# DLR-RM/curvature

Hardware: AMD Instinct MI355X
Metric: KFAC factor-build + invert + sample throughput (higher is better)
Workload: dtype f32

## Files before the change

### curvature_amd/csrc/gemm_nt.h

```cpp
#pragma once
#include "common.h"

namespace curv {

constexpr int GEMM_THREADS = 256;

struct GemmDev {
  const float* A;
  const float* B;
  float* C;
  const float* E;
  const float* F;
  long long a_rs, a_cs;
  long long b_rs, b_cs;
  long long c_rs, c_cs;
  long long e_rs, e_cs;
  long long f_rs, f_cs;
  int M, N, K;
  int epilogue;
  float alpha, beta;
  int tiles_n, tile_base;
  int tm;
  int tri;
  unsigned a_bytes, b_bytes;
// ... 20 lines not shown
typedef __attribute__((address_space(3))) char lds_char_t;

__device__ __forceinline__ void nt_epilogue(const GemmDev& d, int i, int j, float acc) {
  gfl* C = (gfl*)d.C;
  const gfl* E = (const gfl*)d.E;
  const gfl* F = (const gfl*)d.F;
  const int ep = d.epilogue;
  const long long ci = i * d.c_rs + j * d.c_cs;
  float v = d.alpha * acc;
  if (ep == CURV_EPI_SQUARE) v = d.alpha * acc * acc;
  else if (ep == CURV_EPI_MUL_E) v *= E[i * d.e_rs + j * d.e_cs];
  else if (ep == CURV_EPI_ADD_E) v += E[i * d.e_rs + j * d.e_cs];
  else if (ep == CURV_EPI_MUL_E_ADD_F) v = v * E[i * d.e_rs + j * d.e_cs] + F[i * d.f_rs + j * d.f_cs];
  if (d.beta != 0.0f) v += d.beta * C[ci];
  C[ci] = v;
}

__device__ __forceinline__ void gemm_nt_tile(const GemmDev& d, int local, lds_char_t* lds, float* __restrict__ slabs) {
  using namespace nt;
  const int tid = threadIdx.x, lane = tid & 63;
  const int wave = __builtin_amdgcn_readfirstlane(tid >> 6);
  const int r32 = lane & 31, h = lane >> 5;
  const int wm = wave >> 1, wn = wave & 1;
  const bool split = d.n_slices > 1;
  const int item = local;
  int slice = 0;
  if (split) { slice = local % d.n_slices; local /= d.n_slices; }
  int tm = local / d.tiles_n, tn = local - tm * d.tiles_n;
  if (d.tri == CURV_TRI_A_LOWER) tm = (d.M + TM - 1) / TM - 1 - tm;
  else if (d.tri == CURV_TRI_B_UPPER) tn = d.tiles_n - 1 - tn;
  const int i0 = tm * TM, j0 = tn * TM, M = d.M, N = d.N;
  int K = d.K;
  const bool cut = (d.tri == CURV_TRI_A_LOWER && i0 + TM < K) || (d.tri == CURV_TRI_B_UPPER && j0 + TM < K);
  if (d.tri == CURV_TRI_A_LOWER) K = min(K, i0 + TM);
  else if (d.tri == CURV_TRI_B_UPPER) K = min(K, j0 + TM);
  int kb = 0;
  bool inner = false;
  if (split) {
    kb = slice * d.kslice;
    if (kb >= K) return;
    inner = kb + d.kslice < K;
    K = min(K, kb + d.kslice);
  }
  (void)cut; (void)inner;
  const int n_stages = (K - kb + KC - 1) / KC;

  const int rsub = RPP * wave + (lane >> LANES_PER_ROW_SHIFT);
  const int g_lane = (lane & (SLOTS - 1)) ^ ((rsub >> KEY_SHIFT) & (SLOTS - 1));
  int voff_a[PIECES], voff_b[PIECES];
#pragma unroll
  for (int p = 0; p < PIECES; ++p) {
    const int ra = min(i0 + 4 * RPP * p + rsub, M - 1), rb = min(j0 + 4 * RPP * p + rsub, N - 1);
    voff_a[p] = (int)(((long long)ra * d.a_rs + 4 * g_lane) * 4);
    voff_b[p] = (int)(((long long)rb * d.b_cs + 4 * g_lane) * 4);
  }
  const __amdgpu_buffer_rsrc_t rsa = __builtin_amdgcn_make_buffer_rsrc((void*)d.A, 0, d.a_bytes, 0x00020000);
  const __amdgpu_buffer_rsrc_t rsb = __builtin_amdgcn_make_buffer_rsrc((void*)d.B, 0, d.b_bytes, 0x00020000);

  unsigned addr[4][STEPS];
#pragma unroll
  for (int o = 0; o < 4; ++o) {
    const int R = ((o < 2) ? 64 * wm : 64 * wn) + (o & 1) * 32 + r32;
    const unsigned pbase = (o < 2) ? 0u : 2u * PANEL_B;
    const int rkey = (R >> KEY_SHIFT) & (SLOTS - 1);
#pragma unroll
    for (int j = 0; j < STEPS; ++j) addr[o][j] = pbase + R * ROW_B + (((2 * j + h) ^ rkey) << 4);
  }
  f32x16 c00 = {0}, c01 = {0}, c10 = {0}, c11 = {0};

  constexpr int OOB = (int)0x80000000;
  auto issue = [&](int i, bool live, int k0n, unsigned nbuf) {
    const int p = i / PIECES, slot = i % PIECES;
    const unsigned lbase = (p ? 2u * PANEL_B : 0u) + nbuf + (unsigned)(RPP * wave + 4 * RPP * slot) * ROW_B;
    if (p == 0) __builtin_amdgcn_raw_ptr_buffer_load_lds(rsa, (lds_void_t*)(lds + lbase), 16, live ? voff_a[slot] : OOB, k0n * 4, 0, 0);
    else __builtin_amdgcn_raw_ptr_buffer_load_lds(rsb, (lds_void_t*)(lds + lbase), 16, live ? voff_b[slot] : OOB, k0n * 4, 0, 0);
  };
  if (n_stages > 0) {
    const bool live = kb + 4 * g_lane < K;
#pragma unroll
    for (int i = 0; i < NP; ++i) issue(i, live, kb, 0u);
  }
  for (int t = 0; t < n_stages; ++t) {
    __builtin_amdgcn_s_waitcnt(0x0f70);
    __syncthreads();
    const bool more = t + 1 < n_stages;
    const int k0n = kb + (t + 1) * KC;
    const bool live_n = more && k0n + 4 * g_lane < K;
    const unsigned buf = (unsigned)(t & 1) * PANEL_B, nbuf = PANEL_B - buf;
    const int kbase = kb + t * KC;
    const bool tail_stage = kbase + KC > K;
    auto rd = [&](int o, int j) { return *reinterpret_cast<const __attribute__((address_space(3))) f32x4*>(lds + addr[o][j] + buf); };
    auto mask_step = [&](int j, f32x4& xa0, f32x4& xa1, f32x4& xb0, f32x4& xb1) {
      if (tail_stage) {
        asm volatile("; k tail" ::: "memory");
#pragma unroll
        for (int e = 0; e < 4; ++e) {
          const bool gone = kbase + 4 * (2 * j + h) + e >= K;
          xa0[e] = gone ? 0.0f : xa0[e]; xa1[e] = gone ? 0.0f : xa1[e];
          xb0[e] = gone ? 0.0f : xb0[e]; xb1[e] = gone ? 0.0f : xb1[e];
        }
      }
    };
    f32x4 a0 = rd(0, 0), a1 = rd(1, 0), b0 = rd(2, 0), b1 = rd(3, 0);
#pragma unroll
    for (int j = 0; j < STEPS; ++j) {
      mask_step(j, a0, a1, b0, b1);
      f32x4 na0, na1, nb0, nb1;
      if (j + 1 < STEPS) { na0 = rd(0, j + 1); na1 = rd(1, j + 1); nb0 = rd(2, j + 1); nb1 = rd(3, j + 1); }
#pragma unroll
      for (int e = 0; e < 4; ++e) {
        c00 = __builtin_amdgcn_mfma_f32_32x32x2f32(a0[e], b0[e], c00, 0, 0, 0);
        c01 = __builtin_amdgcn_mfma_f32_32x32x2f32(a0[e], b1[e], c01, 0, 0, 0);
        c10 = __builtin_amdgcn_mfma_f32_32x32x2f32(a1[e], b0[e], c10, 0, 0, 0);
        c11 = __builtin_amdgcn_mfma_f32_32x32x2f32(a1[e], b1[e], c11, 0, 0, 0);
        if (e < PPS && PPS * j + e < NP) issue(PPS * j + e, live_n, k0n, nbuf);
      }
      if (j + 1 < STEPS) { a0 = na0; a1 = na1; b0 = nb0; b1 = nb1; }
    }
  }

  if (split) {
    gfl* slab = (gfl*)slabs + d.slab_base + (long long)item * (TM * TM);
    auto store_raw = [&](const f32x16& acc, int m, int n) {
      const int c = 64 * wn + 32 * n + r32;
#pragma unroll
      for (int reg = 0; reg < 16; ++reg) {
        const int r = 64 * wm + 32 * m + (reg & 3) + 8 * (reg >> 2) + 4 * h;
        slab[r * TM + c] = acc[reg];
      }
    };
    store_raw(c00, 0, 0);
    store_raw(c01, 0, 1);
    store_raw(c10, 1, 0);
    store_raw(c11, 1, 1);
// ... 18 lines not shown
```

### curvature_amd/csrc/invert.hip

```cpp
#include <type_traits>
#include "kernarg.h"
#include "mma64.h"
#include <hip/hip_ext.h>

#include <algorithm>
#include <chrono>
#include <cstdlib>
#include <mutex>
#include <vector>

namespace curv {

constexpr int INV_THREADS = MMA_THREADS;
constexpr int SQ_FLAGS = 32;
constexpr int SQ_FD = 0, SQ_FLC = 4, SQ_FLROW = 8, SQ_FT = 12;
constexpr int SQ_SPIN_LIMIT = 1 << 21;
#ifdef CURV_SQ_TRACE
__device__ long long g_sq_trace[256];
#define KT_BEGIN(slot) { if (threadIdx.x == 0 && k0 == 4 * (CURV_SQ_TRACE - 1)) atomicMax((unsigned long long*)&g_sq_trace[slot], (1ull << 62) - (unsigned long long)wall_clock64()); }
#define KT_END(slot) { if (threadIdx.x == 0 && k0 == 4 * (CURV_SQ_TRACE - 1)) atomicMax((unsigned long long*)&g_sq_trace[slot], (unsigned long long)wall_clock64()); }
#define SQT(slot) { if (threadIdx.x == 0 && f == 0 && stamp == CURV_SQ_TRACE) g_sq_trace[slot] = wall_clock64(); }
#define FIT(k) { if (threadIdx.x == 0 && trace_base >= 0) g_sq_trace[trace_base + (k)] = wall_clock64(); }
#else
#define SQT(slot)
// ... 5 lines not shown
#define PQT(slot) { if (threadIdx.x == 0 && blockIdx.x == 0 && k0 == 4 * (CURV_SQ_TRACE - 1)) g_sq_trace[slot] = wall_clock64(); }
#else
#define PQT(slot)
#endif

struct InvDev {
  const float* F;
  float* L;
  double* W;
  double* X;
  int* info;
  int n, np, P;
  float sqrt_s, sqrt_n;
  int reverse;
  int f64_in;
  double* Xout;
  const double* R;
  double* Zm;
  int r_minus, pad_;
  float* C32;
  float* X32;
  float* S32;
  double pivot_min;
};
typedef __attribute__((address_space(1))) float gfloat;
__device__ __host__ __forceinline__ bool s_in_sweep(const InvDev& d) { return d.X32 == nullptr; }
__device__ __host__ __forceinline__ int s_kind(const InvDev& d) { return d.X32 != nullptr ? 0 : (d.Zm != nullptr ? 2 : 1); }

template <typename CountFn>
__device__ __forceinline__ bool locate(const InvDev* __restrict__ t, int nf, int bid, CountFn cnt, int& f,
                                       int& local) {
  const int lane = threadIdx.x & 63;
  int base = 0;
  for (int f0 = 0; f0 < nf; f0 += 64) {
    const int ff = f0 + lane;
    const int c = (ff < nf) ? cnt(t[ff]) : 0;
    int incl = c;
#pragma unroll
    for (int o = 1; o < 64; o <<= 1) {
      const int v = __shfl_up(incl, o, 64);
      if (lane >= o) incl += v;
    }
// ... 1038 lines not shown
  if (local < n_below) panel_quarter_body<true>(d, k0, nb, kend + local, 0, q, Own, Ts);
  else panel_quarter_body<false>(d, k0, nb, 0, local - n_below, q, Own, Ts);
  KT_END(237)
}
__global__ void __launch_bounds__(INV_THREADS, 3)
panel_product_kernel(const InvDev* __restrict__ t, int nf, int k0, int kend) {
  __shared__ double As[NB * OPA], Bs[NB * OPA > OKS * LDA ? NB * OPA : OKS * LDA];
  panel_product_body<2>(t, nf, k0, kend, As, Bs);
}
__global__ void __launch_bounds__(1024)
panel_product_wide_kernel(const InvDev* __restrict__ t, int nf, int k0, int kend) {
  __shared__ double As[NB * OPA], Bs[NB * OPA > OKS * LDA ? NB * OPA : OKS * LDA];
  panel_product_body<4>(t, nf, k0, kend, As, Bs);
}

constexpr int SKS = 32;
constexpr int SPA = SKS + 1;
constexpr int SPB = NB + 32;
struct Tile32 {
  const gbyte* a;
  const gbyte* b;
  gfloat* out;
  int np, ke0, ke1;
  bool a64, b64, accumulate, negate;
};
__device__ __forceinline__ void tile32(const Tile32& o, float* __restrict__ As, float* __restrict__ Bs) {
  const int np = o.np;
  const int tid = threadIdx.x, lane = tid & 63, wave = tid >> 6, wm = wave >> 1, wn = wave & 1;
  const int l32 = lane & 31, h = lane >> 5;
  const long long a_off = (long long)(tid >> 3) * np + 4 * (tid & 7), a_step = 32ll * np;
  const long long b_off = (long long)(tid >> 4) * np + 4 * (tid & 15), b_step = 16ll * np;
  typedef const __attribute__((address_space(1))) f32x4 gf4;
  typedef const __attribute__((address_space(1))) f64x4 gd4;
  f32x4 ra[2], rb[2];
  auto fetch = [&](int ke) __attribute__((always_inline)) {
    if (o.a64) {
#pragma unroll
      for (int u = 0; u < 2; ++u) {
        const f64x4 v = *(gd4*)(o.a + (a_off + u * a_step + ke) * 8);
        ra[u] = f32x4{(float)v[0], (float)v[1], (float)v[2], (float)v[3]};
      }
    } else {
#pragma unroll
      for (int u = 0; u < 2; ++u) ra[u] = *(gf4*)(o.a + (a_off + u * a_step + ke) * 4);
    }
    if (o.b64) {
#pragma unroll
      for (int u = 0; u < 2; ++u) {
        const f64x4 v = *(gd4*)(o.b + (b_off + u * b_step + (long long)ke * np) * 8);
        rb[u] = f32x4{(float)v[0], (float)v[1], (float)v[2], (float)v[3]};
      }
    } else {
#pragma unroll
      for (int u = 0; u < 2; ++u) rb[u] = *(gf4*)(o.b + (b_off + u * b_step + (long long)ke * np) * 4);
    }
  };
  f32x16 acc = {0};
  fetch(o.ke0);
  for (int ke = o.ke0; ke < o.ke1; ke += SKS) {
#pragma unroll
    for (int u = 0; u < 2; ++u)
#pragma unroll
      for (int e = 0; e < 4; ++e) {
        As[((tid >> 3) + 32 * u) * SPA + 4 * (tid & 7) + e] = ra[u][e];
        Bs[((tid >> 4) + 16 * u) * SPB + 4 * (tid & 15) + e] = rb[u][e];
      }
    __syncthreads();
    if (ke + SKS < o.ke1) fetch(ke + SKS);
#pragma unroll
    for (int kk = 0; kk < SKS; kk += 2) {
      const float av = As[(32 * wm + l32) * SPA + kk + h];
      const float bv = Bs[(kk + h) * SPB + 32 * wn + l32];
      acc = __builtin_amdgcn_mfma_f32_32x32x2f32(av, bv, acc, 0, 0, 0);
    }
    __syncthreads();
  }
  gbyte* base = (gbyte*)(o.out + (long long)(32 * wm + 4 * h) * np + 32 * wn + l32);
  if (!o.accumulate) {
#pragma unroll
    for (int reg = 0; reg < 16; ++reg)
      *(gfloat*)(base + (long long)((reg & 3) + 8 * (reg >> 2)) * np * 4) = o.negate ? -acc[reg] : acc[reg];
  } else {
    float old[16];
#pragma unroll
    for (int reg = 0; reg < 16; ++reg) old[reg] = *(const gfloat*)(base + (long long)((reg & 3) + 8 * (reg >> 2)) * np * 4);
#pragma unroll
    for (int reg = 0; reg < 16; ++reg) *(gfloat*)(base + (long long)((reg & 3) + 8 * (reg >> 2)) * np * 4) = old[reg] + acc[reg];
  }
}
__device__ __host__ __forceinline__ long long supd_tiles(int P, int kind, int kend) {
  if (kind != 0 || P <= kend) return 0;
  const long long nsb = (P - kend + SB - 1) / SB, ncb = (kend + SB - 1) / SB;
  return nsb * ncb * (SB * SB);
}
__global__ void __launch_bounds__(INV_THREADS, 3)
supd32_kernel(const InvDev* __restrict__ t, int nf, int k0, int kend, int n_items) {
  __shared__ float As[NB * SPA], Bs[SKS * SPB];
  int item;
  {
    const int bid = blockIdx.x, xcd = bid & 7, jj = bid >> 3;
    item = ((jj / (SB * SB)) * 8 + xcd) * (SB * SB) + (jj % (SB * SB));
  }
  if (item >= n_items) return;
  int f, local;
  if (!locate(t, nf, item, [kend](const InvDev& d) { return (int)supd_tiles(d.P, s_kind(d), kend); }, f, local)) return;
  const InvDev& d = t[f];
  const int np = d.np, r = d.P - kend;
  const int ncb = (kend + SB - 1) / SB;
  const int sb = local / (SB * SB), in = local - sb * (SB * SB);
  const int a = sb / ncb, cb = sb - a * ncb;
  const int ri = a * SB + in / SB, j = cb * SB + in % SB;
  if (ri >= r || j >= kend) return;
  const int i = kend + ri;
  const bool own = j >= k0;
  Tile32 o;
  o.np = np;
  o.a = (const gbyte*)((const gfloat*)d.C32 + (long long)i * NB * np);
  o.a64 = false;
  o.b = own ? (const gbyte*)((const gdouble*)d.X + j * NB) : (const gbyte*)((const gfloat*)d.X32 + j * NB);
  o.b64 = own;
  o.ke0 = (own ? j : k0) * NB;
  o.ke1 = kend * NB;
  o.out = (gfloat*)d.S32 + (long long)i * NB * np + j * NB;
  o.accumulate = !own;
  o.negate = false;
  tile32(o, As, Bs);
}
__device__ __host__ __forceinline__ long long xrow_tiles(int P, int kind, int k0, int kend) {
  if (kind != 0 || P <= k0) return 0;
  return (long long)((kend < P ? kend : P) - k0) * k0;
}
__global__ void __launch_bounds__(INV_THREADS, 3)
xrows32_kernel(const InvDev* __restrict__ t, int nf, int k0, int kend) {
  __shared__ float As[NB * SPA], Bs[SKS * SPB];
  int f, local;
  if (!locate(t, nf, blockIdx.x, [k0, kend](const InvDev& d) { return (int)xrow_tiles(d.P, s_kind(d), k0, kend); }, f, local)) return;
  const InvDev& d = t[f];
  const int np = d.np, nb = (kend < d.P ? kend : d.P) - k0;
  const int j = local / nb, c = nb - 1 - (local - j * nb);
  Tile32 o;
  o.np = np;
  o.a = (const gbyte*)((const gdouble*)d.X + (long long)(k0 + c) * NB * np);
  o.a64 = true;
  o.b = (const gbyte*)((const gfloat*)d.S32 + j * NB);
  o.b64 = false;
  o.ke0 = k0 * NB;
  o.ke1 = (k0 + c + 1) * NB;
  o.out = (gfloat*)d.X32 + (long long)(k0 + c) * NB * np + j * NB;
  o.accumulate = false;
  o.negate = true;
  tile32(o, As, Bs);
}

__global__ void __launch_bounds__(INV_THREADS)
inv_finalize_kernel(const InvDev* __restrict__ t, int nf, int sq) {
  __shared__ float tile[NB][NB + 1];
  int f, local;
  if (!locate(t, nf, blockIdx.x, [](const InvDev& d) { return d.P * d.P; }, f, local)) return;
  const InvDev& d = t[f];
  const int n = d.n, np = d.np, q = d.P;
  const int ti = local / q, tj = local - ti * q;
  const gdouble* X = (const gdouble*)d.X;
  const gfloat* X32 = (const gfloat*)d.X32;
  gfloat* L = (gfloat*)d.L;
  const int w = __builtin_amdgcn_readfirstlane(threadIdx.x >> 6), c = threadIdx.x & 63;
  if (!d.reverse) {
    gdouble* Xo = (gdouble*)d.Xout;
    const gdouble* S = d.Zm != nullptr ? (const gdouble*)d.Zm : X;
#pragma unroll 4
    for (int u = 0; u < 16; ++u) {
      const int i = ti * NB + w + 4 * u, j = tj * NB + c;
      if (i < n && j < n) {
        double v = (j <= i) ? S[(long long)i * np + j] : 0.0;
        if (d.r_minus && j <= i) v = ((const gdouble*)d.R)[(long long)i * n + j] - v;
        Xo[(long long)i * n + j] = v;
      }
    }
    return;
  }
  if (tj > ti) {
#pragma unroll 4
    for (int u = 0; u < 16; ++u) {
      const int i = ti * NB + w + 4 * u, j = tj * NB + c;
      if (i < n && j < n) L[(long long)i * n + j] = 0.0f;
    }
    return;
  }
  double xv[16];
  const int i_l = ti * NB + c;
#pragma unroll
  for (int u = 0; u < 16; ++u) {
    const int j = tj * NB + w + 4 * u;
    const int rs = n - 1 - j, cs = n - 1 - i_l;
    const bool live = i_l < n && j < n && j <= i_l;
    if (X32 == nullptr || rs / sq == cs / sq) xv[u] = live ? X[(long long)rs * np + cs] : 0.0;
    else xv[u] = live ? (double)X32[(long long)rs * np + cs] : 0.0;
  }
#pragma unroll
  for (int u = 0; u < 16; ++u) tile[w + 4 * u][c] = (float)xv[u];
  __syncthreads();
#pragma unroll
  for (int u = 0; u < 16; ++u) {
    const int i = ti * NB + w + 4 * u, j = tj * NB + c;
    if (i < n && j < n) L[(long long)i * n + j] = tile[c][w + 4 * u];
  }
}

constexpr int INV_UPLOAD_CHUNK = 28;

static size_t inv_table_bytes(int n) { return align_up((size_t)std::max(n, 1) * sizeof(InvDev), 256); }
static size_t inv_flags_bytes(int n) { return align_up((size_t)std::max(n, 1) * SQ_FLAGS * sizeof(int), 256); }

struct SideStream {
  hipStream_t stream = nullptr;
  hipEvent_t ev_main[2] = {nullptr, nullptr};
  hipEvent_t ev_side[2] = {nullptr, nullptr};
  hipEvent_t ev_tail = nullptr;
};
struct StreamSet {
  SideStream side[2];
  hipStream_t aux = nullptr;
  hipStream_t masked = nullptr;
  hipEvent_t ev_fork = nullptr, ev_join = nullptr, ev_join2 = nullptr;
  hipEvent_t ev_chain[2] = {nullptr, nullptr};
};
// ... 78 lines not shown
extern "C" int curv_debug_sq_trace(long long* out) {
  return hipMemcpyFromSymbol(out, HIP_SYMBOL(curv::g_sq_trace), 256 * sizeof(long long)) == hipSuccess ? 0 : 1;
}
#endif

extern "C" int curv_init_streams(void) {
  StreamSet* ss = nullptr;
  return stream_set(&ss);
}

extern "C" size_t curv_chol_inv_workspace_bytes(const curv_inv_desc* descs, int n_factors) {
  size_t total = 2 * inv_table_bytes(n_factors) + 2 * inv_flags_bytes(n_factors);
  for (int i = 0; i < n_factors; ++i) {
    if (descs[i].n <= 0) return 0;
    const size_t np = (size_t)cdiv(descs[i].n, NB) * NB;
    total += 2 * np * np * sizeof(double) + 3 * np * np * sizeof(float);
  }
  return total;
}

static int sweep_nbo(bool latency_bound) { return latency_bound ? 4 : 6; }
struct GroupSweep {
  hipStream_t stream;
  SideStream* side;
  const std::vector<InvDev>* tabp;
  InvDev* table;
  int* flags;
  bool latency_bound;
  int n_factors = 0, Pmax = 0, NBO = 4, k0 = 0, panel = 0;
  long long fin_tiles = 0, quarter_prod = 0;
  bool use_square = false, far_pending = false, inv_pending = false, capturing = false;
// ... 60 lines not shown
    }
    auto launch_product = [&](hipStream_t st, long long jobs, hipEvent_t done) -> int {
      const InvDev* tb = table;
      if (jobs <= quarter_prod)
        hipExtLaunchKernelGGL(panel_product_quarter_kernel, dim3((unsigned)(cdivll(jobs, 8) * 32)), dim3(INV_THREADS), 0, st,
                              nullptr, done, 0, tb, n_factors, k0, kend);
      else if (jobs <= WIDE_PROD)
        hipExtLaunchKernelGGL(panel_product_wide_kernel, dim3((unsigned)jobs), dim3(1024), 0, st, nullptr, done, 0, tb, n_factors,
                              k0, kend);
      else
        hipExtLaunchKernelGGL(panel_product_kernel, dim3((unsigned)jobs), dim3(INV_THREADS), 0, st, nullptr, done, 0, tb,
                              n_factors, k0, kend);
      CURV_LAUNCH_CHECK();
      return CURV_OK;
    };
    long long inv_jobs = 0, inv_tiles = 0;
    for (const InvDev& d : tab) {
      prod_tiles += panel_jobs(d.P, s_kind(d), k0, kend);
      inv_jobs += xrow_tiles(d.P, s_kind(d), k0, kend);
      inv_tiles += supd_tiles(d.P, s_kind(d), kend);
    }
    bool fork_recorded = false;
    if (prod_tiles > 0) {
      fork_recorded = !capturing;
      const int rc = launch_product(stream, prod_tiles, fork_recorded ? side->ev_main[panel & 1] : nullptr);
      if (rc != CURV_OK) return rc;
    }
    long long near_tiles = 0, far_tiles = 0;
    for (const InvDev& d : tab) {
      near_tiles += strip_tiles(d.P, kend, kend, row0, s_in_sweep(d));
      far_tiles += outer_tiles(d.P, kend, row0, s_in_sweep(d));
    }
    hipStream_t inv_st = side->stream;
    const bool inv_work = inv_jobs > 0 || inv_tiles > 0;
    const bool side_work = far_tiles > 0 || inv_work;
    if (side_work) {
      if (!fork_recorded) CURV_HIP_CHECK(hipEventRecord(side->ev_main[panel & 1], stream));
      CURV_HIP_CHECK(hipStreamWaitEvent(side->stream, side->ev_main[panel & 1], 0));
    }
    if (near_tiles > 0) {
      if (far_pending) {
        CURV_HIP_CHECK(hipStreamWaitEvent(stream, side->ev_side[(panel + 1) & 1], 0));
      }
      far_pending = false;
      if (near_tiles <= WIDE_NEAR)
        hipLaunchKernelGGL(outer_update_wide_kernel, dim3((unsigned)near_tiles), dim3(1024), 0, stream, table, n_factors,
                           k0, kend, kend, row0, 1, (int)near_tiles);
      else
        hipLaunchKernelGGL(outer_update_kernel, dim3((unsigned)near_tiles), dim3(INV_THREADS), 0, stream, table, n_factors, k0,
// ... 9 lines not shown
      if (trail > 0) {
        const long long g1 = cdivll(trail, 8 * SB * SB) * 8 * SB * SB;
        hipExtLaunchKernelGGL(outer_update_dma_kernel, dim3((unsigned)g1), dim3(INV_THREADS), 0, side->stream, nullptr,
                              (ride && s_tiles == 0) ? side->ev_side[panel & 1] : nullptr, 0, tb, n_factors, k0, kend, row0, (int)trail);
        CURV_LAUNCH_CHECK();
      }
      if (s_tiles > 0) {
        const long long g2 = cdivll(s_tiles, 8 * SB * SB) * 8 * SB * SB;
        hipExtLaunchKernelGGL(outer_update_kernel, dim3((unsigned)g2), dim3(INV_THREADS), 0, side->stream, nullptr,
                              ride ? side->ev_side[panel & 1] : nullptr, 0, tb, n_factors, k0, kend, row0, 0, 2, (int)s_tiles);
        CURV_LAUNCH_CHECK();
      }
      if (!ride) CURV_HIP_CHECK(hipEventRecord(side->ev_side[panel & 1], side->stream));
      far_pending = true;
    }
    if (inv_jobs > 0) {
      hipLaunchKernelGGL(xrows32_kernel, dim3((unsigned)inv_jobs), dim3(INV_THREADS), 0, inv_st, table, n_factors, k0, kend);
      CURV_LAUNCH_CHECK();
      inv_pending = true;
    }
    if (inv_tiles > 0) {
      const long long grid = cdivll(inv_tiles, 8 * SB * SB) * 8 * SB * SB;
      hipLaunchKernelGGL(supd32_kernel, dim3((unsigned)grid), dim3(INV_THREADS), 0, inv_st, table, n_factors, k0, kend,
                         (int)inv_tiles);
      CURV_LAUNCH_CHECK();
      inv_pending = true;
    }
    k0 += NBO;
    ++panel;
    return CURV_OK;
  }

  int end(hipEvent_t chain_done = nullptr) {
    if (chain_done != nullptr) CURV_HIP_CHECK(hipEventRecord(chain_done, stream));
    if (far_pending) CURV_HIP_CHECK(hipStreamWaitEvent(stream, side->ev_side[(panel + 1) & 1], 0));
    if (inv_pending) {
      CURV_HIP_CHECK(hipEventRecord(side->ev_tail, side->stream));
      CURV_HIP_CHECK(hipStreamWaitEvent(stream, side->ev_tail, 0));
    }
    hipLaunchKernelGGL(inv_finalize_kernel, dim3((unsigned)fin_tiles), dim3(INV_THREADS), 0, stream, table, n_factors, NBO * NB);
    CURV_LAUNCH_CHECK();
    return CURV_OK;
  }
};

static int chol_sweep_group(hipStream_t stream, SideStream* side, const std::vector<InvDev>& tab, InvDev* table, int* flags,
                            bool latency_bound, hipEvent_t chain_done = nullptr) {
  GroupSweep g(stream, side, tab, table, flags, latency_bound);
  int rc = g.begin();
  while (rc == CURV_OK && !g.done()) rc = g.panel_step();
  return rc == CURV_OK ? g.end(chain_done) : rc;
}

constexpr int SPLIT_P = 16;

// ... 1 lines not shown

static int await_verdict(const EarlyStatus* early) {
  if (early != nullptr) CURV_HIP_CHECK(hipEventSynchronize(early->ev));
  return CURV_OK;
}

static int chol_sweep(hipStream_t stream, std::vector<InvDev>& tab, void* workspace, size_t workspace_bytes,
                      const char* who, const EarlyStatus* early = nullptr) {
  const int n_factors = (int)tab.size();
  static const int latency_max = getenv("CURV_LATENCY_MAX") ? atoi(getenv("CURV_LATENCY_MAX")) : 64;
  bool any_rhs = false;
  for (const InvDev& d : tab) any_rhs = any_rhs || d.R != nullptr;
  const bool latency_bound = n_factors <= latency_max && !any_rhs;
  size_t need = 2 * inv_table_bytes(n_factors) + 2 * inv_flags_bytes(n_factors);
  for (const InvDev& d : tab)
    need += (d.R != nullptr ? 3 : 2) * (size_t)d.np * d.np * sizeof(double) + (d.reverse ? 3 * (size_t)d.np * d.np * sizeof(float) : 0);
  if (workspace == nullptr || workspace_bytes < need) {
    set_error("%s: workspace too small (%zu < %zu bytes)", who, workspace_bytes, need);
    return CURV_ERR_WORKSPACE;
  }
  char* p = reinterpret_cast<char*>(workspace) + 2 * inv_table_bytes(n_factors);
  int* flags0 = reinterpret_cast<int*>(p);
  int* flags1 = reinterpret_cast<int*>(p + inv_flags_bytes(n_factors));
  p += 2 * inv_flags_bytes(n_factors);
  std::vector<InvDev> big, small;
  int Pmax = 0;
  for (const InvDev& d : tab) Pmax = std::max(Pmax, d.P);
  const int split = std::max(SPLIT_P, Pmax / 2);
  for (InvDev& d : tab) {
    d.W = reinterpret_cast<double*>(p); p += (size_t)d.np * d.np * sizeof(double);
    d.X = reinterpret_cast<double*>(p); p += (size_t)d.np * d.np * sizeof(double);
    if (d.R != nullptr) { d.Zm = reinterpret_cast<double*>(p); p += (size_t)d.np * d.np * sizeof(double); }
    if (d.reverse) {
      d.C32 = reinterpret_cast<float*>(p); p += (size_t)d.np * d.np * sizeof(float);
      d.X32 = reinterpret_cast<float*>(p); p += (size_t)d.np * d.np * sizeof(float);
      d.S32 = reinterpret_cast<float*>(p); p += (size_t)d.np * d.np * sizeof(float);
    }
    (d.P > split || latency_bound ? big : small).push_back(d);
  }
  StreamSet* ss = nullptr;
  { const int rc = stream_set(&ss); if (rc != CURV_OK) return rc; }
  InvDev* table0 = reinterpret_cast<InvDev*>(workspace);
  InvDev* table1 = reinterpret_cast<InvDev*>(reinterpret_cast<char*>(workspace) + inv_table_bytes(n_factors));
  hipStreamCaptureStatus capture = hipStreamCaptureStatusNone;
  CURV_HIP_CHECK(hipStreamIsCapturing(stream, &capture));
  if (capture != hipStreamCaptureStatusNone) {
    if (early != nullptr) {
      set_error("%s: the early status read-back is a host copy and cannot be captured", who);
      return CURV_ERR_INVALID;
    }
    if (!big.empty()) {
// ... 144 lines not shown
```

Before: 4204.

## Reuse NT MFMA GEMM stage loop for f32 inverse panel updates

Pulls the double-buffered DMA-to-LDS MFMA stage loop out of the NT GEMM into a shared helper. The inverse's row and Schur-update kernels (tile32-based xrows32/supd32) are replaced with 128x128 NT tiles that work on transposed f32 copies (XT32, ST32), with XCD-aware block ordering. A new xsq32 kernel converts and transposes each diagonal block square into an extra f32 buffer. The finalize kernel now reads the transposed f32 inverse directly, dropping its LDS transpose. The aim is to replace the small 64x64 tiles that use scalar LDS staging with the faster GEMM engine, at the cost of an extra kernel launch and more workspace.

New measurement: 4166. About the same (-0.9%).

```diff
diff --git a/curvature_amd/csrc/gemm_nt.h b/curvature_amd/csrc/gemm_nt.h
--- a/curvature_amd/csrc/gemm_nt.h
+++ b/curvature_amd/csrc/gemm_nt.h
@@ -58,6 +58,85 @@
   else if (ep == CURV_EPI_MUL_E_ADD_F) v = v * E[i * d.e_rs + j * d.e_cs] + F[i * d.f_rs + j * d.f_cs];
   if (d.beta != 0.0f) v += d.beta * C[ci];
   C[ci] = v;
+}
+
+__device__ __forceinline__ void nt_dma_lane(int wave, int lane, int& rsub, int& g_lane) {
+  using namespace nt;
+  rsub = RPP * wave + (lane >> LANES_PER_ROW_SHIFT);
+  g_lane = (lane & (SLOTS - 1)) ^ ((rsub >> KEY_SHIFT) & (SLOTS - 1));
+}
+
+__device__ __forceinline__ void nt_stage_loop(const __amdgpu_buffer_rsrc_t rsa, const __amdgpu_buffer_rsrc_t rsb,
+                                              const int (&voff_a)[nt::PIECES], const int (&voff_b)[nt::PIECES], int g_lane,
+                                              int kb, int K, lds_char_t* lds, f32x16& c00, f32x16& c01, f32x16& c10,
+                                              f32x16& c11) {
+  using namespace nt;
+  const int tid = threadIdx.x, lane = tid & 63;
+  const int wave = __builtin_amdgcn_readfirstlane(tid >> 6);
+  const int r32 = lane & 31, h = lane >> 5;
+  const int wm = wave >> 1, wn = wave & 1;
+  const int n_stages = (K - kb + KC - 1) / KC;
+  unsigned addr[4][STEPS];
+#pragma unroll
+  for (int o = 0; o < 4; ++o) {
+    const int R = ((o < 2) ? 64 * wm : 64 * wn) + (o & 1) * 32 + r32;
+    const unsigned pbase = (o < 2) ? 0u : 2u * PANEL_B;
+    const int rkey = (R >> KEY_SHIFT) & (SLOTS - 1);
+#pragma unroll
+    for (int j = 0; j < STEPS; ++j) addr[o][j] = pbase + R * ROW_B + (((2 * j + h) ^ rkey) << 4);
+  }
+  c00 = f32x16{0}; c01 = f32x16{0}; c10 = f32x16{0}; c11 = f32x16{0};
+
+  constexpr int OOB = (int)0x80000000;
+  auto issue = [&](int i, bool live, int k0n, unsigned nbuf) {
+    const int p = i / PIECES, slot = i % PIECES;
+    const unsigned lbase = (p ? 2u * PANEL_B : 0u) + nbuf + (unsigned)(RPP * wave + 4 * RPP * slot) * ROW_B;
+    if (p == 0) __builtin_amdgcn_raw_ptr_buffer_load_lds(rsa, (lds_void_t*)(lds + lbase), 16, live ? voff_a[slot] : OOB, k0n * 4, 0, 0);
+    else __builtin_amdgcn_raw_ptr_buffer_load_lds(rsb, (lds_void_t*)(lds + lbase), 16, live ? voff_b[slot] : OOB, k0n * 4, 0, 0);
+  };
+  if (n_stages > 0) {
+    const bool live = kb + 4 * g_lane < K;
+#pragma unroll
+    for (int i = 0; i < NP; ++i) issue(i, live, kb, 0u);
+  }
+  for (int t = 0; t < n_stages; ++t) {
+    __builtin_amdgcn_s_waitcnt(0x0f70);
+    __syncthreads();
+    const bool more = t + 1 < n_stages;
+    const int k0n = kb + (t + 1) * KC;
+    const bool live_n = more && k0n + 4 * g_lane < K;
+    const unsigned buf = (unsigned)(t & 1) * PANEL_B, nbuf = PANEL_B - buf;
+    const int kbase = kb + t * KC;
+    const bool tail_stage = kbase + KC > K;
+    auto rd = [&](int o, int j) { return *reinterpret_cast<const __attribute__((address_space(3))) f32x4*>(lds + addr[o][j] + buf); };
+    auto mask_step = [&](int j, f32x4& xa0, f32x4& xa1, f32x4& xb0, f32x4& xb1) {
+      if (tail_stage) {
+        asm volatile("; k tail" ::: "memory");
+#pragma unroll
+        for (int e = 0; e < 4; ++e) {
+          const bool gone = kbase + 4 * (2 * j + h) + e >= K;
+          xa0[e] = gone ? 0.0f : xa0[e]; xa1[e] = gone ? 0.0f : xa1[e];
+          xb0[e] = gone ? 0.0f : xb0[e]; xb1[e] = gone ? 0.0f : xb1[e];
+        }
+      }
+    };
+    f32x4 a0 = rd(0, 0), a1 = rd(1, 0), b0 = rd(2, 0), b1 = rd(3, 0);
+#pragma unroll
+    for (int j = 0; j < STEPS; ++j) {
+      mask_step(j, a0, a1, b0, b1);
+      f32x4 na0, na1, nb0, nb1;
+      if (j + 1 < STEPS) { na0 = rd(0, j + 1); na1 = rd(1, j + 1); nb0 = rd(2, j + 1); nb1 = rd(3, j + 1); }
+#pragma unroll
+      for (int e = 0; e < 4; ++e) {
+        c00 = __builtin_amdgcn_mfma_f32_32x32x2f32(a0[e], b0[e], c00, 0, 0, 0);
+        c01 = __builtin_amdgcn_mfma_f32_32x32x2f32(a0[e], b1[e], c01, 0, 0, 0);
+        c10 = __builtin_amdgcn_mfma_f32_32x32x2f32(a1[e], b0[e], c10, 0, 0, 0);
+        c11 = __builtin_amdgcn_mfma_f32_32x32x2f32(a1[e], b1[e], c11, 0, 0, 0);
+        if (e < PPS && PPS * j + e < NP) issue(PPS * j + e, live_n, k0n, nbuf);
+      }
+      if (j + 1 < STEPS) { a0 = na0; a1 = na1; b0 = nb0; b1 = nb1; }
+    }
+  }
 }
 
 __device__ __forceinline__ void gemm_nt_tile(const GemmDev& d, int local, lds_char_t* lds, float* __restrict__ slabs) {
@@ -87,10 +166,8 @@
     K = min(K, kb + d.kslice);
   }
   (void)cut; (void)inner;
-  const int n_stages = (K - kb + KC - 1) / KC;
-
-  const int rsub = RPP * wave + (lane >> LANES_PER_ROW_SHIFT);
-  const int g_lane = (lane & (SLOTS - 1)) ^ ((rsub >> KEY_SHIFT) & (SLOTS - 1));
+  int rsub, g_lane;
+  nt_dma_lane(wave, lane, rsub, g_lane);
   int voff_a[PIECES], voff_b[PIECES];
 #pragma unroll
   for (int p = 0; p < PIECES; ++p) {
@@ -101,67 +178,8 @@
   const __amdgpu_buffer_rsrc_t rsa = __builtin_amdgcn_make_buffer_rsrc((void*)d.A, 0, d.a_bytes, 0x00020000);
   const __amdgpu_buffer_rsrc_t rsb = __builtin_amdgcn_make_buffer_rsrc((void*)d.B, 0, d.b_bytes, 0x00020000);
 
-  unsigned addr[4][STEPS];
-#pragma unroll
-  for (int o = 0; o < 4; ++o) {
-    const int R = ((o < 2) ? 64 * wm : 64 * wn) + (o & 1) * 32 + r32;
-    const unsigned pbase = (o < 2) ? 0u : 2u * PANEL_B;
-    const int rkey = (R >> KEY_SHIFT) & (SLOTS - 1);
-#pragma unroll
-    for (int j = 0; j < STEPS; ++j) addr[o][j] = pbase + R * ROW_B + (((2 * j + h) ^ rkey) << 4);
-  }
-  f32x16 c00 = {0}, c01 = {0}, c10 = {0}, c11 = {0};
-
-  constexpr int OOB = (int)0x80000000;
-  auto issue = [&](int i, bool live, int k0n, unsigned nbuf) {
-    const int p = i / PIECES, slot = i % PIECES;
-    const unsigned lbase = (p ? 2u * PANEL_B : 0u) + nbuf + (unsigned)(RPP * wave + 4 * RPP * slot) * ROW_B;
-    if (p == 0) __builtin_amdgcn_raw_ptr_buffer_load_lds(rsa, (lds_void_t*)(lds + lbase), 16, live ? voff_a[slot] : OOB, k0n * 4, 0, 0);
-    else __builtin_amdgcn_raw_ptr_buffer_load_lds(rsb, (lds_void_t*)(lds + lbase), 16, live ? voff_b[slot] : OOB, k0n * 4, 0, 0);
-  };
-  if (n_stages > 0) {
-    const bool live = kb + 4 * g_lane < K;
-#pragma unroll
-    for (int i = 0; i < NP; ++i) issue(i, live, kb, 0u);
-  }
-  for (int t = 0; t < n_stages; ++t) {
-    __builtin_amdgcn_s_waitcnt(0x0f70);
-    __syncthreads();
-    const bool more = t + 1 < n_stages;
-    const int k0n = kb + (t + 1) * KC;
-    const bool live_n = more && k0n + 4 * g_lane < K;
-    const unsigned buf = (unsigned)(t & 1) * PANEL_B, nbuf = PANEL_B - buf;
-    const int kbase = kb + t * KC;
-    const bool tail_stage = kbase + KC > K;
-    auto rd = [&](int o, int j) { return *reinterpret_cast<const __attribute__((address_space(3))) f32x4*>(lds + addr[o][j] + buf); };
-    auto mask_step = [&](int j, f32x4& xa0, f32x4& xa1, f32x4& xb0, f32x4& xb1) {
-      if (tail_stage) {
-        asm volatile("; k tail" ::: "memory");
-#pragma unroll
-        for (int e = 0; e < 4; ++e) {
-          const bool gone = kbase + 4 * (2 * j + h) + e >= K;
-          xa0[e] = gone ? 0.0f : xa0[e]; xa1[e] = gone ? 0.0f : xa1[e];
-          xb0[e] = gone ? 0.0f : xb0[e]; xb1[e] = gone ? 0.0f : xb1[e];
-        }
-      }
-    };
-    f32x4 a0 = rd(0, 0), a1 = rd(1, 0), b0 = rd(2, 0), b1 = rd(3, 0);
-#pragma unroll
-    for (int j = 0; j < STEPS; ++j) {
-      mask_step(j, a0, a1, b0, b1);
-      f32x4 na0, na1, nb0, nb1;
-      if (j + 1 < STEPS) { na0 = rd(0, j + 1); na1 = rd(1, j + 1); nb0 = rd(2, j + 1); nb1 = rd(3, j + 1); }
-#pragma unroll
-      for (int e = 0; e < 4; ++e) {
-        c00 = __builtin_amdgcn_mfma_f32_32x32x2f32(a0[e], b0[e], c00, 0, 0, 0);
-        c01 = __builtin_amdgcn_mfma_f32_32x32x2f32(a0[e], b1[e], c01, 0, 0, 0);
-        c10 = __builtin_amdgcn_mfma_f32_32x32x2f32(a1[e], b0[e], c10, 0, 0, 0);
-        c11 = __builtin_amdgcn_mfma_f32_32x32x2f32(a1[e], b1[e], c11, 0, 0, 0);
-        if (e < PPS && PPS * j + e < NP) issue(PPS * j + e, live_n, k0n, nbuf);
-      }
-      if (j + 1 < STEPS) { a0 = na0; a1 = na1; b0 = nb0; b1 = nb1; }
-    }
-  }
+  f32x16 c00, c01, c10, c11;
+  nt_stage_loop(rsa, rsb, voff_a, voff_b, g_lane, kb, K, lds, c00, c01, c10, c11);
 
   if (split) {
     gfl* slab = (gfl*)slabs + d.slab_base + (long long)item * (TM * TM);
diff --git a/curvature_amd/csrc/invert.hip b/curvature_amd/csrc/invert.hip
--- a/curvature_amd/csrc/invert.hip
+++ b/curvature_amd/csrc/invert.hip
@@ -1,4 +1,5 @@
 #include <type_traits>
+#include "gemm_nt.h"
 #include "kernarg.h"
 #include "mma64.h"
 #include <hip/hip_ext.h>
@@ -43,18 +44,21 @@
   float sqrt_s, sqrt_n;
   int reverse;
   int f64_in;
-  double* Xout;
+  union {
+    double* Xout;
+    float* Xsq32;
+  };
   const double* R;
   double* Zm;
   int r_minus, pad_;
   float* C32;
-  float* X32;
-  float* S32;
+  float* XT32;
+  float* ST32;
   double pivot_min;
 };
 typedef __attribute__((address_space(1))) float gfloat;
-__device__ __host__ __forceinline__ bool s_in_sweep(const InvDev& d) { return d.X32 == nullptr; }
-__device__ __host__ __forceinline__ int s_kind(const InvDev& d) { return d.X32 != nullptr ? 0 : (d.Zm != nullptr ? 2 : 1); }
+__device__ __host__ __forceinline__ bool s_in_sweep(const InvDev& d) { return d.XT32 == nullptr; }
+__device__ __host__ __forceinline__ int s_kind(const InvDev& d) { return d.XT32 != nullptr ? 0 : (d.Zm != nullptr ? 2 : 1); }
 
 template <typename CountFn>
 __device__ __forceinline__ bool locate(const InvDev* __restrict__ t, int nf, int bid, CountFn cnt, int& f,
@@ -1123,154 +1127,160 @@
   panel_product_body<4>(t, nf, k0, kend, As, Bs);
 }
 
-constexpr int SKS = 32;
-constexpr int SPA = SKS + 1;
-constexpr int SPB = NB + 32;
-struct Tile32 {
-  const gbyte* a;
-  const gbyte* b;
-  gfloat* out;
-  int np, ke0, ke1;
-  bool a64, b64, accumulate, negate;
+namespace inv32 {
+constexpr int TB = nt::TM / NB;
+constexpr int XCH = 8;
+enum { STORE = 0, STORE_NEG = 1, ADD = 2 };
+struct Panel {
+  const float* base;
+  int pitch;
+  int rows;
+  int row_floats;
 };
-__device__ __forceinline__ void tile32(const Tile32& o, float* __restrict__ As, float* __restrict__ Bs) {
-  const int np = o.np;
-  const int tid = threadIdx.x, lane = tid & 63, wave = tid >> 6, wm = wave >> 1, wn = wave & 1;
-  const int l32 = lane & 31, h = lane >> 5;
-  const long long a_off = (long long)(tid >> 3) * np + 4 * (tid & 7), a_step = 32ll * np;
-  const long long b_off = (long long)(tid >> 4) * np + 4 * (tid & 15), b_step = 16ll * np;
-  typedef const __attribute__((address_space(1))) f32x4 gf4;
-  typedef const __attribute__((address_space(1))) f64x4 gd4;
-  f32x4 ra[2], rb[2];
-  auto fetch = [&](int ke) __attribute__((always_inline)) {
-    if (o.a64) {
-#pragma unroll
-      for (int u = 0; u < 2; ++u) {
-        const f64x4 v = *(gd4*)(o.a + (a_off + u * a_step + ke) * 8);
-        ra[u] = f32x4{(float)v[0], (float)v[1], (float)v[2], (float)v[3]};
-      }
-    } else {
-#pragma unroll
-      for (int u = 0; u < 2; ++u) ra[u] = *(gf4*)(o.a + (a_off + u * a_step + ke) * 4);
-    }
-    if (o.b64) {
-#pragma unroll
-      for (int u = 0; u < 2; ++u) {
-        const f64x4 v = *(gd4*)(o.b + (b_off + u * b_step + (long long)ke * np) * 8);
-        rb[u] = f32x4{(float)v[0], (float)v[1], (float)v[2], (float)v[3]};
-      }
-    } else {
-#pragma unroll
-      for (int u = 0; u < 2; ++u) rb[u] = *(gf4*)(o.b + (b_off + u * b_step + (long long)ke * np) * 4);
-    }
+}
+__device__ __forceinline__ int inv32_item() {
+  const int bid = blockIdx.x, xcd = bid & 7, jj = bid >> 3;
+  return ((jj / inv32::XCH) * 8 + xcd) * inv32::XCH + jj % inv32::XCH;
+}
+static long long inv32_grid(long long items) { return cdivll(items, 8 * inv32::XCH) * 8 * inv32::XCH; }
+__device__ __forceinline__ void inv32_tile(const inv32::Panel& rows, const inv32::Panel& cols, int kb, int K,
+                                           gfloat* __restrict__ out, int out_pitch, int mode, lds_char_t* lds) {
+  using namespace nt;
+  const int tid = threadIdx.x, lane = tid & 63;
+  const int wave = __builtin_amdgcn_readfirstlane(tid >> 6);
+  const int r32 = lane & 31, h = lane >> 5, wm = wave >> 1, wn = wave & 1;
+  int rsub, g_lane;
+  nt_dma_lane(wave, lane, rsub, g_lane);
+  int voff_a[PIECES], voff_b[PIECES];
+#pragma unroll
+  for (int p = 0; p < PIECES; ++p) {
+    const int ra = min(4 * RPP * p + rsub, cols.rows - 1), rb = min(4 * RPP * p + rsub, rows.rows - 1);
+    voff_a[p] = (ra * cols.pitch + 4 * g_lane) * 4;
+    voff_b[p] = (rb * rows.pitch + 4 * g_lane) * 4;
+  }
+  const unsigned a_bytes = (unsigned)(((long long)(cols.rows - 1) * cols.pitch + cols.row_floats) * 4);
+  const unsigned b_bytes = (unsigned)(((long long)(rows.rows - 1) * rows.pitch + rows.row_floats) * 4);
+  const __amdgpu_buffer_rsrc_t rsa = __builtin_amdgcn_make_buffer_rsrc((void*)cols.base, 0, a_bytes, 0x00020000);
+  const __amdgpu_buffer_rsrc_t rsb = __builtin_amdgcn_make_buffer_rsrc((void*)rows.base, 0, b_bytes, 0x00020000);
+  f32x16 c00, c01, c10, c11;
+  nt_stage_loop(rsa, rsb, voff_a, voff_b, g_lane, kb, K, lds, c00, c01, c10, c11);
+  typedef __attribute__((address_space(1))) f32x4 gf4;
+  auto put = [&](const f32x16& acc, int m, int n) {
+    const int c = 64 * wm + 32 * m + 4 * h;
+    if (64 * wm + 32 * m >= cols.rows) return;
+    gfloat* p = out + (long long)(64 * wn + 32 * n + r32) * out_pitch + c;
+    f32x4 v[4];
+#pragma unroll
+    for (int g = 0; g < 4; ++g) v[g] = f32x4{acc[4 * g], acc[4 * g + 1], acc[4 * g + 2], acc[4 * g + 3]};
+    if (mode == inv32::ADD) {
+      f32x4 old[4];
+#pragma unroll
+      for (int g = 0; g < 4; ++g) old[g] = *(const gf4*)(p + 8 * g);
+#pragma unroll
+      for (int g = 0; g < 4; ++g) v[g] = old[g] + v[g];
+    } else if (mode == inv32::STORE_NEG) {
+#pragma unroll
+      for (int g = 0; g < 4; ++g) v[g] = -v[g];
+    }
+#pragma unroll
+    for (int g = 0; g < 4; ++g) *(gf4*)(p + 8 * g) = v[g];
   };
-  f32x16 acc = {0};
-  fetch(o.ke0);
-  for (int ke = o.ke0; ke < o.ke1; ke += SKS) {
-#pragma unroll
-    for (int u = 0; u < 2; ++u)
-#pragma unroll
-      for (int e = 0; e < 4; ++e) {
-        As[((tid >> 3) + 32 * u) * SPA + 4 * (tid & 7) + e] = ra[u][e];
-        Bs[((tid >> 4) + 16 * u) * SPB + 4 * (tid & 15) + e] = rb[u][e];
-      }
-    __syncthreads();
-    if (ke + SKS < o.ke1) fetch(ke + SKS);
-#pragma unroll
-    for (int kk = 0; kk < SKS; kk += 2) {
-      const float av = As[(32 * wm + l32) * SPA + kk + h];
-      const float bv = Bs[(kk + h) * SPB + 32 * wn + l32];
-      acc = __builtin_amdgcn_mfma_f32_32x32x2f32(av, bv, acc, 0, 0, 0);
-    }
-    __syncthreads();
-  }
-  gbyte* base = (gbyte*)(o.out + (long long)(32 * wm + 4 * h) * np + 32 * wn + l32);
-  if (!o.accumulate) {
-#pragma unroll
-    for (int reg = 0; reg < 16; ++reg)
-      *(gfloat*)(base + (long long)((reg & 3) + 8 * (reg >> 2)) * np * 4) = o.negate ? -acc[reg] : acc[reg];
-  } else {
-    float old[16];
-#pragma unroll
-    for (int reg = 0; reg < 16; ++reg) old[reg] = *(const gfloat*)(base + (long long)((reg & 3) + 8 * (reg >> 2)) * np * 4);
-#pragma unroll
-    for (int reg = 0; reg < 16; ++reg) *(gfloat*)(base + (long long)((reg & 3) + 8 * (reg >> 2)) * np * 4) = old[reg] + acc[reg];
-  }
-}
+  put(c00, 0, 0);
+  put(c01, 0, 1);
+  put(c10, 1, 0);
+  put(c11, 1, 1);
+}
+
+__device__ __host__ __forceinline__ int xsq_blocks(int P, int kind, int k0, int kend) {
+  if (kind != 0 || P <= k0) return 0;
+  const int nb = (kend < P ? kend : P) - k0;
+  return nb * nb;
+}
+__device__ __host__ __forceinline__ int xsq_pitch(int np, int k0, int kend) { return np < (kend - k0) * NB ? np : (kend - k0) * NB; }
+__global__ void __launch_bounds__(INV_THREADS)
+xsq32_kernel(const InvDev* __restrict__ t, int nf, int k0, int kend) {
+  __shared__ float tile[NB][NB + 1];
+  int f, local;
+  if (!locate(t, nf, blockIdx.x, [k0, kend](const InvDev& d) { return xsq_blocks(d.P, s_kind(d), k0, kend); }, f, local)) return;
+  const InvDev& d = t[f];
+  const int np = d.np, nb = (kend < d.P ? kend : d.P) - k0, sqp = xsq_pitch(np, k0, kend);
+  const int r = local / nb, c = local - r * nb;
+  const int w = __builtin_amdgcn_readfirstlane(threadIdx.x >> 6), l = threadIdx.x & 63;
+  const gdouble* X = (const gdouble*)d.X + ((long long)(k0 + r) * NB) * np + (k0 + c) * NB;
+  gfloat* sq = (gfloat*)d.Xsq32 + (long long)r * NB * sqp + c * NB;
+  gfloat* xt = (gfloat*)d.XT32 + ((long long)(k0 + c) * NB) * np + (k0 + r) * NB;
+  float v[16];
+#pragma unroll
+  for (int u = 0; u < 16; ++u) v[u] = r >= c ? (float)X[(long long)(w + 4 * u) * np + l] : 0.0f;
+#pragma unroll
+  for (int u = 0; u < 16; ++u) {
+    sq[(w + 4 * u) * sqp + l] = v[u];
+    tile[w + 4 * u][l] = v[u];
+  }
+  __syncthreads();
+#pragma unroll
+  for (int u = 0; u < 16; ++u) xt[(long long)(w + 4 * u) * np + l] = tile[l][w + 4 * u];
+}
+
+__device__ __host__ __forceinline__ long long xleft_tiles(int P, int kind, int k0, int kend) {
+  if (kind != 0 || P <= k0) return 0;
+  const int nb = (kend < P ? kend : P) - k0;
+  return (long long)(k0 / inv32::TB) * ((nb + inv32::TB - 1) / inv32::TB);
+}
+__global__ void __launch_bounds__(INV_THREADS, nt::WGS)
+xleft_nt_kernel(const InvDev* __restrict__ t, int nf, int k0, int kend, int n_items) {
+  __shared__ __attribute__((aligned(1024))) char smem[nt::LDS_B];
+  const int item = inv32_item();
+  if (item >= n_items) return;
+  int f, local;
+  if (!locate(t, nf, item, [k0, kend](const InvDev& d) { return (int)xleft_tiles(d.P, s_kind(d), k0, kend); }, f, local)) return;
+  const InvDev& d = t[f];
+  const int np = d.np, nb = (kend < d.P ? kend : d.P) - k0, sqp = xsq_pitch(np, k0, kend);
+  const int tiles_m = k0 / inv32::TB, tiles_n = (nb + inv32::TB - 1) / inv32::TB;
+  const int tn = tiles_n - 1 - local / tiles_m, tm = local % tiles_m;
+  const int j0 = tm * nt::TM, c0 = tn * nt::TM, width = nb * NB;
+  inv32::Panel rows, cols;
+  rows.base = d.ST32 + (long long)j0 * np + k0 * NB;
+  rows.pitch = np; rows.rows = nt::TM; rows.row_floats = np - k0 * NB;
+  cols.base = d.Xsq32 + (long long)c0 * sqp;
+  cols.pitch = sqp; cols.rows = min(nt::TM, width - c0); cols.row_floats = sqp;
+  inv32_tile(rows, cols, 0, min(width, c0 + nt::TM), (gfloat*)d.XT32 + (long long)j0 * np + k0 * NB + c0, np, inv32::STORE_NEG,
+             (lds_char_t*)smem);
+}
+
 __device__ __host__ __forceinline__ long long supd_tiles(int P, int kind, int kend) {
   if (kind != 0 || P <= kend) return 0;
-  const long long nsb = (P - kend + SB - 1) / SB, ncb = (kend + SB - 1) / SB;
-  return nsb * ncb * (SB * SB);
-}
-__global__ void __launch_bounds__(INV_THREADS, 3)
-supd32_kernel(const InvDev* __restrict__ t, int nf, int k0, int kend, int n_items) {
-  __shared__ float As[NB * SPA], Bs[SKS * SPB];
-  int item;
-  {
-    const int bid = blockIdx.x, xcd = bid & 7, jj = bid >> 3;
-    item = ((jj / (SB * SB)) * 8 + xcd) * (SB * SB) + (jj % (SB * SB));
-  }
+  return (long long)(kend / inv32::TB) * ((P - kend + inv32::TB - 1) / inv32::TB);
+}
+__global__ void __launch_bounds__(INV_THREADS, nt::WGS)
+supd_nt_kernel(const InvDev* __restrict__ t, int nf, int k0, int kend, int n_items) {
+  __shared__ __attribute__((aligned(1024))) char smem[nt::LDS_B];
+  const int item = inv32_item();
   if (item >= n_items) return;
   int f, local;
   if (!locate(t, nf, item, [kend](const InvDev& d) { return (int)supd_tiles(d.P, s_kind(d), kend); }, f, local)) return;
   const InvDev& d = t[f];
-  const int np = d.np, r = d.P - kend;
-  const int ncb = (kend + SB - 1) / SB;
-  const int sb = local / (SB * SB), in = local - sb * (SB * SB);
-  const int a = sb / ncb, cb = sb - a * ncb;
-  const int ri = a * SB + in / SB, j = cb * SB + in % SB;
-  if (ri >= r || j >= kend) return;
-  const int i = kend + ri;
-  const bool own = j >= k0;
-  Tile32 o;
-  o.np = np;
-  o.a = (const gbyte*)((const gfloat*)d.C32 + (long long)i * NB * np);
-  o.a64 = false;
-  o.b = own ? (const gbyte*)((const gdouble*)d.X + j * NB) : (const gbyte*)((const gfloat*)d.X32 + j * NB);
-  o.b64 = own;
-  o.ke0 = (own ? j : k0) * NB;
-  o.ke1 = kend * NB;
-  o.out = (gfloat*)d.S32 + (long long)i * NB * np + j * NB;
-  o.accumulate = !own;
-  o.negate = false;
-  tile32(o, As, Bs);
-}
-__device__ __host__ __forceinline__ long long xrow_tiles(int P, int kind, int k0, int kend) {
-  if (kind != 0 || P <= k0) return 0;
-  return (long long)((kend < P ? kend : P) - k0) * k0;
-}
-__global__ void __launch_bounds__(INV_THREADS, 3)
-xrows32_kernel(const InvDev* __restrict__ t, int nf, int k0, int kend) {
-  __shared__ float As[NB * SPA], Bs[SKS * SPB];
-  int f, local;
-  if (!locate(t, nf, blockIdx.x, [k0, kend](const InvDev& d) { return (int)xrow_tiles(d.P, s_kind(d), k0, kend); }, f, local)) return;
-  const InvDev& d = t[f];
-  const int np = d.np, nb = (kend < d.P ? kend : d.P) - k0;
-  const int j = local / nb, c = nb - 1 - (local - j * nb);
-  Tile32 o;
-  o.np = np;
-  o.a = (const gbyte*)((const gdouble*)d.X + (long long)(k0 + c) * NB * np);
-  o.a64 = true;
-  o.b = (const gbyte*)((const gfloat*)d.S32 + j * NB);
-  o.b64 = false;
-  o.ke0 = k0 * NB;
-  o.ke1 = (k0 + c + 1) * NB;
-  o.out = (gfloat*)d.X32 + (long long)(k0 + c) * NB * np + j * NB;
-  o.accumulate = false;
-  o.negate = true;
-  tile32(o, As, Bs);
+  const int np = d.np, tiles_m = kend / inv32::TB;
+  const int tn = local / tiles_m, tm = local - tn * tiles_m;
+  const int j0 = tm * nt::TM, i0 = kend * NB + tn * nt::TM;
+  const bool own = j0 >= k0 * NB;
+  inv32::Panel rows, cols;
+  rows.base = d.XT32 + (long long)j0 * np;
+  rows.pitch = np; rows.rows = nt::TM; rows.row_floats = np;
+  cols.base = d.C32 + (long long)i0 * np;
+  cols.pitch = np; cols.rows = min(nt::TM, np - i0); cols.row_floats = np;
+  inv32_tile(rows, cols, own ? j0 : k0 * NB, kend * NB, (gfloat*)d.ST32 + (long long)j0 * np + i0, np,
+             own ? inv32::STORE : inv32::ADD, (lds_char_t*)smem);
 }
 
 __global__ void __launch_bounds__(INV_THREADS)
-inv_finalize_kernel(const InvDev* __restrict__ t, int nf, int sq) {
-  __shared__ float tile[NB][NB + 1];
+inv_finalize_kernel(const InvDev* __restrict__ t, int nf) {
   int f, local;
   if (!locate(t, nf, blockIdx.x, [](const InvDev& d) { return d.P * d.P; }, f, local)) return;
   const InvDev& d = t[f];
   const int n = d.n, np = d.np, q = d.P;
   const int ti = local / q, tj = local - ti * q;
   const gdouble* X = (const gdouble*)d.X;
-  const gfloat* X32 = (const gfloat*)d.X32;
   gfloat* L = (gfloat*)d.L;
   const int w = __builtin_amdgcn_readfirstlane(threadIdx.x >> 6), c = threadIdx.x & 63;
   if (!d.reverse) {
@@ -1295,29 +1305,24 @@
     }
     return;
   }
-  double xv[16];
-  const int i_l = ti * NB + c;
-#pragma unroll
-  for (int u = 0; u < 16; ++u) {
-    const int j = tj * NB + w + 4 * u;
-    const int rs = n - 1 - j, cs = n - 1 - i_l;
-    const bool live = i_l < n && j < n && j <= i_l;
-    if (X32 == nullptr || rs / sq == cs / sq) xv[u] = live ? X[(long long)rs * np + cs] : 0.0;
-    else xv[u] = live ? (double)X32[(long long)rs * np + cs] : 0.0;
-  }
-#pragma unroll
-  for (int u = 0; u < 16; ++u) tile[w + 4 * u][c] = (float)xv[u];
-  __syncthreads();
+  const gfloat* XT = (const gfloat*)d.XT32;
+  float xv[16];
 #pragma unroll
   for (int u = 0; u < 16; ++u) {
     const int i = ti * NB + w + 4 * u, j = tj * NB + c;
-    if (i < n && j < n) L[(long long)i * n + j] = tile[c][w + 4 * u];
+    xv[u] = (i < n && j <= i) ? XT[(long long)(n - 1 - i) * np + (n - 1 - j)] : 0.0f;
+  }
+#pragma unroll
+  for (int u = 0; u < 16; ++u) {
+    const int i = ti * NB + w + 4 * u, j = tj * NB + c;
+    if (i < n && j < n) L[(long long)i * n + j] = xv[u];
   }
 }
 
 constexpr int INV_UPLOAD_CHUNK = 28;
 
 static size_t inv_table_bytes(int n) { return align_up((size_t)std::max(n, 1) * sizeof(InvDev), 256); }
+static size_t inv_xsq_bytes(int np) { const size_t e = (size_t)std::min(np, 6 * NB); return e * e * sizeof(float); }
 static size_t inv_flags_bytes(int n) { return align_up((size_t)std::max(n, 1) * SQ_FLAGS * sizeof(int), 256); }
 
 struct SideStream {
@@ -1426,7 +1431,7 @@
   for (int i = 0; i < n_factors; ++i) {
     if (descs[i].n <= 0) return 0;
     const size_t np = (size_t)cdiv(descs[i].n, NB) * NB;
-    total += 2 * np * np * sizeof(double) + 3 * np * np * sizeof(float);
+    total += 2 * np * np * sizeof(double) + 3 * np * np * sizeof(float) + inv_xsq_bytes((int)np);
   }
   return total;
 }
@@ -1517,10 +1522,11 @@
       CURV_LAUNCH_CHECK();
       return CURV_OK;
     };
-    long long inv_jobs = 0, inv_tiles = 0;
+    long long sq_jobs = 0, inv_jobs = 0, inv_tiles = 0;
     for (const InvDev& d : tab) {
       prod_tiles += panel_jobs(d.P, s_kind(d), k0, kend);
-      inv_jobs += xrow_tiles(d.P, s_kind(d), k0, kend);
+      sq_jobs += xsq_blocks(d.P, s_kind(d), k0, kend);
+      inv_jobs += xleft_tiles(d.P, s_kind(d), k0, kend);
       inv_tiles += supd_tiles(d.P, s_kind(d), kend);
     }
     bool fork_recorded = false;
@@ -1535,7 +1541,7 @@
       far_tiles += outer_tiles(d.P, kend, row0, s_in_sweep(d));
     }
     hipStream_t inv_st = side->stream;
-    const bool inv_work = inv_jobs > 0 || inv_tiles > 0;
+    const bool inv_work = sq_jobs > 0 || inv_jobs > 0 || inv_tiles > 0;
     const bool side_work = far_tiles > 0 || inv_work;
     if (side_work) {
       if (!fork_recorded) CURV_HIP_CHECK(hipEventRecord(side->ev_main[panel & 1], stream));
@@ -1575,17 +1581,20 @@
       if (!ride) CURV_HIP_CHECK(hipEventRecord(side->ev_side[panel & 1], side->stream));
       far_pending = true;
     }
-    if (inv_jobs > 0) {
-      hipLaunchKernelGGL(xrows32_kernel, dim3((unsigned)inv_jobs), dim3(INV_THREADS), 0, inv_st, table, n_factors, k0, kend);
+    if (sq_jobs > 0) {
+      hipLaunchKernelGGL(xsq32_kernel, dim3((unsigned)sq_jobs), dim3(INV_THREADS), 0, inv_st, table, n_factors, k0, kend);
       CURV_LAUNCH_CHECK();
       inv_pending = true;
     }
+    if (inv_jobs > 0) {
+      hipLaunchKernelGGL(xleft_nt_kernel, dim3((unsigned)inv32_grid(inv_jobs)), dim3(INV_THREADS), 0, inv_st, table, n_factors,
+                         k0, kend, (int)inv_jobs);
+      CURV_LAUNCH_CHECK();
+    }
     if (inv_tiles > 0) {
-      const long long grid = cdivll(inv_tiles, 8 * SB * SB) * 8 * SB * SB;
-      hipLaunchKernelGGL(supd32_kernel, dim3((unsigned)grid), dim3(INV_THREADS), 0, inv_st, table, n_factors, k0, kend,
-                         (int)inv_tiles);
+      hipLaunchKernelGGL(supd_nt_kernel, dim3((unsigned)inv32_grid(inv_tiles)), dim3(INV_THREADS), 0, inv_st, table, n_factors,
+                         k0, kend, (int)inv_tiles);
       CURV_LAUNCH_CHECK();
-      inv_pending = true;
     }
     k0 += NBO;
     ++panel;
@@ -1599,7 +1608,7 @@
       CURV_HIP_CHECK(hipEventRecord(side->ev_tail, side->stream));
       CURV_HIP_CHECK(hipStreamWaitEvent(stream, side->ev_tail, 0));
     }
-    hipLaunchKernelGGL(inv_finalize_kernel, dim3((unsigned)fin_tiles), dim3(INV_THREADS), 0, stream, table, n_factors, NBO * NB);
+    hipLaunchKernelGGL(inv_finalize_kernel, dim3((unsigned)fin_tiles), dim3(INV_THREADS), 0, stream, table, n_factors);
     CURV_LAUNCH_CHECK();
     return CURV_OK;
   }
@@ -1631,7 +1640,7 @@
   const bool latency_bound = n_factors <= latency_max && !any_rhs;
   size_t need = 2 * inv_table_bytes(n_factors) + 2 * inv_flags_bytes(n_factors);
   for (const InvDev& d : tab)
-    need += (d.R != nullptr ? 3 : 2) * (size_t)d.np * d.np * sizeof(double) + (d.reverse ? 3 * (size_t)d.np * d.np * sizeof(float) : 0);
+    need += (d.R != nullptr ? 3 : 2) * (size_t)d.np * d.np * sizeof(double) + (d.reverse ? 3 * (size_t)d.np * d.np * sizeof(float) + inv_xsq_bytes(d.np) : 0);
   if (workspace == nullptr || workspace_bytes < need) {
     set_error("%s: workspace too small (%zu < %zu bytes)", who, workspace_bytes, need);
     return CURV_ERR_WORKSPACE;
@@ -1650,8 +1659,9 @@
     if (d.R != nullptr) { d.Zm = reinterpret_cast<double*>(p); p += (size_t)d.np * d.np * sizeof(double); }
     if (d.reverse) {
       d.C32 = reinterpret_cast<float*>(p); p += (size_t)d.np * d.np * sizeof(float);
-      d.X32 = reinterpret_cast<float*>(p); p += (size_t)d.np * d.np * sizeof(float);
-      d.S32 = reinterpret_cast<float*>(p); p += (size_t)d.np * d.np * sizeof(float);
+      d.XT32 = reinterpret_cast<float*>(p); p += (size_t)d.np * d.np * sizeof(float);
+      d.ST32 = reinterpret_cast<float*>(p); p += (size_t)d.np * d.np * sizeof(float);
+      d.Xsq32 = reinterpret_cast<float*>(p); p += inv_xsq_bytes(d.np);
     }
     (d.P > split || latency_bound ? big : small).push_back(d);
   }
```
